# sahaRatul/sela

Hardware: AMD Instinct MI355X
Metric: Msamples/s encode+decode, 16-bit stereo 44.1kHz, 1/2/4/8 GPU; bit-exact vs CPU (higher is better)
Workload: dtype f64+int64

## Files before the change

### sela_amd/csrc/sela_encode.hip

```cpp
#include <algorithm>
#include <atomic>
#include <random>
#include <vector>

#include "sela_device.h"

namespace sela {

constexpr int kPadC = 64;
constexpr int kHalfEntries = kBlock / 4;
constexpr int kParityLen = kPadC + kHalfEntries + 64;
constexpr int kLastT0 = (kHalfEntries + 64) / 32 - 1;
constexpr int kFirstT1 = (kHalfEntries - kPadC) / 32;
constexpr int kRingHalf = 64;
constexpr int kRingLen = 2 * kRingHalf + 64;
constexpr int kRingsPerXcd = 512;
constexpr int kXcds = 8;
constexpr int kPadS = 128;
constexpr int kSBufWords = (kPadS + kBlock) / 32 * 33;
constexpr int kSmallBase = 8992;
constexpr int kBigBytes = kSmallBase + 3008;
static_assert(kResWordsCap * 4 <= kSmallBase, "packed residue words must fit the dead sample buffer");
static_assert(kSBufWords * 4 <= kSmallBase && kSmallBase % 16 == 0, "sample buffer must end below the analysis arrays");
static_assert(kBigBytes >= 2 * kParityLen * 8, "the FP64 parity arrays must fit");
// ... 877 lines not shown
    const int lane = threadIdx.x;

    const uint32_t e = blockIdx.x - n_workers;
    uint32_t frame, sig;
    block_of(e, n_sig, frame, sig);
    if (frame >= n_frames)
        return;
    const uint32_t block_id = frame * n_sig + sig;
    uint32_t flags = 0;
    if (kFused && fa.pcm_ready && !await_frame(fa.pcm_ready, pcm, frame, ticket, fa.nap_limit))
        flags |= SELA_HIP_FLAG_INTERNAL;

    double* const E = reinterpret_cast<double*>(big) + kPadC;
    double* const O = reinterpret_cast<double*>(big) + kParityLen + kPadC;
    double* const E1 = E - kHalfEntries;
    double* const O1 = O - kHalfEntries;
    SmallArrays* const sm = reinterpret_cast<SmallArrays*>(big + kSmallBase);

    int32_t s[kPerLane];
    {
        const int16_t* fp = pcm_after_wait(pcm) + (size_t)frame * kBlock * channels;
        if (channels == 2) {
            const uint32_t* fp2 = reinterpret_cast<const uint32_t*>(fp);
            uint32_t w[kPerLane];
#pragma unroll
            for (int t = 0; t < kPerLane; t++) {
                w[t] = (kFused && fa.pcm_ready) ? load_through(fp2 + lane + 64 * t) : fp2[lane + 64 * t];
            }
            unpack_stereo<kPerLane>(sig, w, s);
        } else {
            const int16_t* const ps = fp + (size_t)lane * channels + sig;
#pragma unroll
            for (int t = 0; t < kPerLane; t++)
                s[t] = ps[(uint32_t)(64 * t) * channels];
        }
    }

    double* const mine = (lane & 1) ? O : E;
    double* const mine1 = (lane & 1) ? O1 : E1;
    const int half = lane >> 1;
    double mean = 0.0;
    bool have_mean = false;
    if (e >= self_blocks) {
        for (uint32_t spin = 0; spin < kMeanWaitSpins; spin++) {
            if (__hip_atomic_load(mean_ready + e, __ATOMIC_RELAXED, __HIP_MEMORY_SCOPE_AGENT) == fa.tag) {
                __builtin_amdgcn_fence(__ATOMIC_ACQUIRE, "workgroup");
                have_mean = true;
                break;
            }
            __builtin_amdgcn_s_sleep(16);
        }
        if (have_mean)
            mean = __builtin_bit_cast(double, __hip_atomic_load(reinterpret_cast<uint64_t*>(mean_out) + e, __ATOMIC_RELAXED, __HIP_MEMORY_SCOPE_AGENT));
        have_mean = __builtin_amdgcn_readfirstlane((int)have_mean) != 0;
        mean = read_first_lane(mean);
    }
    SELA_STAMP(1);
    if (!have_mean) {
    for (int m = lane; m < kPadC; m += 64) {
        E[m - kPadC] = 0.0;
        O[m - kPadC] = 0.0;
    }
#pragma unroll
    for (int t = 0; t <= kLastT0; t++)
        mine[half + 32 * t] = scale_sample(s[t]);
    wave_sync();

    __builtin_amdgcn_s_setprio(3);
    double sum = 0.0;
#pragma unroll 1
    for (int h = 0; h < 2; h++) {
        if (h == 1) {
            wave_sync();
#pragma unroll
            for (int t = kFirstT1; t < kPerLane; t++)
                mine1[half + 32 * t] = scale_sample(s[t]);
            wave_sync();
        }
        uint32_t addr = (uint32_t)(uintptr_t)(__attribute__((address_space(3))) double*)E;
        MeanFetch f0, f1;
        SELA_MEAN_ISSUE(f0, addr, 0, sum);
#pragma unroll 1
        for (int m0 = 0; m0 < kHalfEntries; m0 += 16) {
            mean_wait(f0, sum);
            SELA_MEAN_ISSUE(f1, addr, 64, sum);
            mean_steps(f0, sum);
            mean_wait(f1, sum);
            SELA_MEAN_ISSUE(f0, addr, 128, sum);
            mean_steps(f1, sum);
            addr += 128;
        }
        mean_wait(f0, sum);
    }
    mean = sum / (double)kBlock;
    __builtin_amdgcn_s_setprio(0);
    }

    SELA_STAMP(2);
    wave_sync();
    for (int m = lane; m < kPadC; m += 64) {
        E[m - kPadC] = 0.0;
        O[m - kPadC] = 0.0;
    }
#pragma unroll
    for (int t = 0; t <= kLastT0; t++)
        mine[half + 32 * t] = scale_sample(s[t]) - mean;
    wave_sync();

    SELA_STAMP(3);
    double acc_e = 0.0, acc_o = 0.0;
    {
        uint32_t xcc;
        asm volatile("s_getreg_b32 %0, hwreg(HW_REG_XCC_ID)" : "=s"(xcc));
        xcc &= kXcds - 1;
        uint32_t* const pool = ring_owner + xcc * kRingsPerXcd;
        uint32_t slot = 0;
        if (lane == 0) {
            slot = (e >> 3) & (kRingsPerXcd - 1);
            while (atomicExch(pool + slot, ticket) == ticket)
                slot = (slot + 1) & (kRingsPerXcd - 1);
        }
        slot = (uint32_t)__builtin_amdgcn_readfirstlane((int)slot);
        double* const ring = reinterpret_cast<double*>(
            read_first_lane((uint64_t)(rings + ((size_t)xcc * kRingsPerXcd + slot) * kRingLen)));
        __attribute__((address_space(1))) double* const ring_g = (__attribute__((address_space(1))) double*)ring;
        auto store_chunk = [&](int k, const double* resident) {
#pragma unroll
            for (int t = 0; t < kRingHalf / 64; t++) {
                const double c = resident[half + 32 * (t + (kRingHalf / 64) * k)];
                ring_g[(k & 1) * kRingHalf + lane + 64 * t] = c;
                if (t == 0 && !(k & 1) && lane < 16)
                    ring_g[2 * kRingHalf + lane] = c;
            }
        };
        store_chunk(0, mine);
        store_chunk(1, mine);
        asm volatile("s_waitcnt vmcnt(0)\n\ts_dcache_inv" ::: "memory");

        double A = E[-lane];
        double B = 0.0;
        uint32_t addr_e = (uint32_t)(uintptr_t)(__attribute__((address_space(3))) double*)(E - lane);
        uint32_t addr_o = (uint32_t)(uintptr_t)(__attribute__((address_space(3))) double*)(O - lane);
        const double* c_ptr = ring;
        AcFetch f0, f1;
        asm volatile("" : "+v"(A));
        SELA_AC_ISSUE_S(f0, c_ptr, 0, 64, acc_e, acc_o);
        SELA_AC_ISSUE_V(f0, addr_e, addr_o, 0, 1, 2, 3, 4, 5, 6, 7, 8, acc_e, acc_o);
        constexpr int kSwitch = kBlock / 2 / kRingHalf;
        const bool falling = !kFused && n_workers == 0 && fa.priorities != 0;
#pragma unroll 1
        for (int k = 0; k < kBlock / kRingHalf; k++) {
            if (falling && k == 0)
                __builtin_amdgcn_s_setprio(2);
            if (falling && k == kSwitch)
                __builtin_amdgcn_s_setprio(1);
            if (k == kSwitch) {
                wave_sync();
#pragma unroll
                for (int t = kFirstT1; t < kPerLane; t++)
                    mine1[half + 32 * t] = scale_sample(s[t]) - mean;
                wave_sync();
                addr_e -= kHalfEntries * 8;
                addr_o -= kHalfEntries * 8;
            }
            if (k >= 1 && k + 1 < kBlock / kRingHalf)
                store_chunk(k + 1, k >= kSwitch ? mine1 : mine);
#pragma unroll 1
            for (int it = 0; it < kRingHalf / 32; it++) {
                if (it == kRingHalf / 32 - 1)
                    asm volatile("s_waitcnt vmcnt(0)\n\ts_dcache_inv" ::: "memory");
                ac_wait(f0, acc_e, acc_o);
                SELA_AC_ISSUE_S(f1, c_ptr, 128, 192, acc_e, acc_o);
                ac_steps_head(f0, A, B, acc_e, acc_o);
                SELA_AC_ISSUE_V(f1, addr_e, addr_o, 8, 9, 10, 11, 12, 13, 14, 15, 16, acc_e, acc_o);
                ac_steps_tail(f0, A, B, acc_e, acc_o);
                ac_wait(f1, acc_e, acc_o);
                SELA_AC_ISSUE_S(f0, c_ptr, 256, 320, acc_e, acc_o);
                ac_steps_head(f1, A, B, acc_e, acc_o);
                SELA_AC_ISSUE_V(f0, addr_e, addr_o, 16, 17, 18, 19, 20, 21, 22, 23, 24, acc_e, acc_o);
                ac_steps_tail(f1, A, B, acc_e, acc_o);
                c_ptr += 32;
                addr_e += 128;
                addr_o += 128;
            }
            if (k & 1)
                c_ptr = ring;
        }
        ac_wait(f0, acc_e, acc_o);
        if (lane == 0)
            atomicExch(pool + slot, 0u);
    }
    wave_sync();

    SELA_STAMP(4);
    {
        const double ac0 = read_first_lane(acc_e);
        if (lane <= 50) {
            sm->ac[2 * lane] = lane == 0 ? 1.0 : acc_e / ac0;
            sm->ac[2 * lane + 1] = acc_o / ac0;
        }
    }
    wave_sync();

    double k_lo = 0.0, k_hi = 0.0;
    if (!kFused && n_workers == 0 && fa.priorities != 0)
        __builtin_amdgcn_s_setprio(1);
    else
        __builtin_amdgcn_s_setprio(2);
    {
        double g0a = sm->ac[lane + 1], g1a = g0a;
        double g0b = lane < 36 ? sm->ac[lane + 65] : 0.0, g1b = g0b;
        double err = 1.0;
        double g = read_first_lane(g1a);
        double ki = -g / err;
        err += g * ki;
        sm->k[0] = ki;
        constexpr int kTwoRegs = kMaxOrder - 64 + 1;
#pragma unroll 1
        for (int i = 1; i < kTwoRegs; i++) {
            const double sa = wave_shl1(read_first_lane(g1b), g1a);
            const double sb = wave_shl1_zero(g1b);
            g1a = sa + ki * g0a;
            g0a = sa * ki + g0a;
            g1b = sb + ki * g0b;
            g0b = sb * ki + g0b;
            g = read_first_lane(g1a);
            ki = -g / err;
            err += g * ki;
            sm->k[i] = ki;
        }
#pragma unroll 1
        for (int i = kTwoRegs; i < kMaxOrder; i++) {
            const double sa = wave_shl1_zero(g1a);
            g1a = sa + ki * g0a;
            g0a = sa * ki + g0a;
            g = read_first_lane(g1a);
            ki = -g / err;
            err += g * ki;
            sm->k[i] = ki;
        }
        wave_sync();
        k_lo = sm->k[lane];
        k_hi = lane < kMaxOrder - 64 ? sm->k[lane + 64] : 0.0;
        wave_sync();
    }
    if (kMode == 3) {
        uint64_t h_ac = hash_term(sm->ac[lane], lane) ^ (lane + 64 <= kMaxOrder ? hash_term(sm->ac[lane + 64], lane + 64) : 0ull);
        uint64_t h_k = hash_term(k_lo, lane) ^ (lane < kMaxOrder - 64 ? hash_term(k_hi, lane + 64) : 0ull);
        h_ac = lanes_xor<64>(h_ac);
        h_k = lanes_xor<64>(h_k);
        if (lane == 0) {
            uint64_t* const hp = reinterpret_cast<uint64_t*>(trace) + 2 * (size_t)block_id;
            hp[0] = h_ac;
            hp[1] = h_k;
        }
    }

    {
        constexpr bool kAcInLds = true;
        uint64_t* const sizes_pub = fa.sizes_pub;
        const uint64_t sizes_tag = fa.sizes_tag;
#define SELA_TAIL_TRACE_RESIDUES fa.trace_residues
#include "sela_encode_tail.inc"
#undef SELA_TAIL_TRACE_RESIDUES
    }
    SELA_STAMP(12);
    if (kFused) {
        const uint32_t g = frame / kGroupFrames;
        const uint32_t blocks_in_group = min((uint32_t)kGroupFrames, n_frames - g * kGroupFrames) * n_sig;
        stores_done();
        uint32_t last = 0;
        if (lane == 0)
            last = group_arrive(fa.group_count + (size_t)g * kGroupCountStride, fa.tag, blocks_in_group) ? 1u : 0u;
        if (__builtin_amdgcn_readfirstlane((int)last)) {
            drop_stale_lines();
            finish_group(fa, g, lane);
        }
    }
    SELA_STAMP(13);
    if (kMode == 2 && lane == 0)
        for (int i = 0; i < 13; i++)
            phase_cycles[(size_t)block_id * 16 + i] = (uint64_t)(stamp[i + 1] - stamp[i]);
}

constexpr int kTeamMirror = 24;
constexpr int kTeamWin = 16;
constexpr int kTeamAhead = 3;
constexpr int kTeamMeanChunk = 64;

template <int P>
struct TeamPlan {
    static constexpr int B = kWave / P;
    static constexpr int G = (kMaxOrder + 1 + P - 1) / P;
    static constexpr int kChunk = P == 8 ? 16 : 64;
    static constexpr int kRing = P == 8 ? 160 : 256;
    static constexpr int kStride = P == 8 ? kRing + kTeamMirror : kRing + 48;
    static constexpr int kPer = kChunk / P;
    static constexpr int kMeanPer = kTeamMeanChunk / P;
    static constexpr int kRingBytes = B * kStride * 8;
    static constexpr int kCwBase = kBigBytes;
    static constexpr int kKStride = 104;
    static constexpr int kQBase = kSmallBase;
    static constexpr int kQStride = 104;
    static constexpr int kLdsBytes = kRingBytes > kCwBase + kCoefWordsCap * 4 ? kRingBytes : kCwBase + kCoefWordsCap * 4;
    static_assert(G + kTeamAhead <= kTeamWin && kChunk % kTeamWin == 0 && kRing % kChunk == 0 && kStride % 32 == (P == 8 ? 24 : 16) && kStride >= kRing + kTeamMirror, "team plan");
    static_assert((G * P - 1) + kChunk + kChunk <= kRing && 2 * kTeamMeanChunk <= kRing, "the ring must hold the lags' reach, the chunk in use and the chunk being written");
    static_assert(kLdsBytes * 12 <= 160 * 1024, "twelve waves per CU");
    static_assert(B * kKStride * 8 <= kQBase && B * kKStride * 8 <= kRingBytes && B * kQStride <= 104 * 8, "k[] in the dead rings below the q store; the q store inside SmallArrays::ac");
};

template <int P>
__device__ __forceinline__ uint32_t team_first(uint32_t v)
{
    if constexpr (P == 16) {
        return (uint32_t)__builtin_amdgcn_mov_dpp((int)v, 0x150 , 0xf, 0xf, true);
    } else {
        static_assert(P == 8, "teams of 8 or 16 lanes");
        const int q = __builtin_amdgcn_mov_dpp((int)v, 0x00 , 0xf, 0xf, true);
        return (uint32_t)__builtin_amdgcn_update_dpp(q, q, 0x114 , 0xf, 0xa , false);
    }
}
template <int P>
__device__ __forceinline__ double team_first(double v)
{
    const uint64_t x = __builtin_bit_cast(uint64_t, v);
    return __builtin_bit_cast(double, ((uint64_t)team_first<P>((uint32_t)(x >> 32)) << 32) | team_first<P>((uint32_t)x));
}

template <int kPer, int kStep>
__device__ __forceinline__ void team_load_raw(const int16_t* __restrict__ fp, uint32_t channels, uint32_t sig, int first, int32_t (&raw)[kPer])
{
    if (channels == 2) {
        const uint32_t* pw = reinterpret_cast<const uint32_t*>(fp) + first;
        uint32_t w[kPer];
        if constexpr (kStep == 1 && kPer % 4 == 0) {
#pragma unroll
            for (int u = 0; u < kPer / 4; u++) {
                const uint4 v = reinterpret_cast<const uint4*>(pw)[u];
                w[4 * u] = v.x, w[4 * u + 1] = v.y, w[4 * u + 2] = v.z, w[4 * u + 3] = v.w;
            }
        } else if constexpr (kStep == 1 && kPer % 2 == 0) {
#pragma unroll
            for (int u = 0; u < kPer / 2; u++) {
                const uint2 v = reinterpret_cast<const uint2*>(pw)[u];
                w[2 * u] = v.x, w[2 * u + 1] = v.y;
            }
        } else {
#pragma unroll
            for (int u = 0; u < kPer; u++)
                w[u] = pw[u * kStep];
        }
        if constexpr (kStep == 1) {
            const uint32_t first_shift = sig == 1 ? 16u : 0u;
            const uint32_t second_mask = sig == 2 ? 0xFFFFFFFFu : 0u;
#pragma unroll
            for (int i = 0; i < kPer; i++) {
                const int32_t a = (int32_t)(w[i] << (16 - first_shift)) >> 16, b = ((int32_t)w[i] >> 16) & (int32_t)second_mask;
                raw[i] = a - b;
            }
        } else {
            unpack_stereo<kPer>(sig, w, raw);
        }
    } else {
        const int16_t* const ps = fp + (size_t)first * channels + sig;
#pragma unroll
        for (int i = 0; i < kPer; i++)
            raw[i] = ps[(uint32_t)(i * kStep) * channels];
    }
}

template <int kPer, int kStep, bool kStereo>
__device__ __forceinline__ void team_fetch(const int16_t* __restrict__ fp, uint32_t channels, uint32_t sig, int first, uint32_t (&w)[kPer])
{
    if constexpr (kStereo) {
        const uint32_t* pw = reinterpret_cast<const uint32_t*>(fp) + first;
#pragma unroll
        for (int u = 0; u < kPer; u++)
            w[u] = pw[u * kStep];
    } else {
        const int16_t* const ps = fp + (size_t)first * channels + sig;
#pragma unroll
        for (int i = 0; i < kPer; i++)
            w[i] = (uint32_t)(int32_t)ps[(uint32_t)(i * kStep) * channels];
    }
}
template <int kPer, bool kStereo>
__device__ __forceinline__ void team_unpack(uint32_t sig, const uint32_t (&w)[kPer], int32_t (&raw)[kPer])
{
    if constexpr (kStereo) {
        unpack_stereo<kPer>(sig, w, raw);
    } else {
#pragma unroll
        for (int i = 0; i < kPer; i++)
            raw[i] = (int32_t)w[i];
    }
}

template <int kPer, int kStep, bool kCentre, bool kMirror, int kRing>
__device__ __forceinline__ void team_stage(double* ring_b, int pos, const int32_t (&raw)[kPer], double mean)
{
#pragma unroll
    for (int i = 0; i < kPer; i++) {
        const double x = scale_sample(raw[i]);
        const double c = kCentre ? x - mean : x;
        ring_b[pos + i * kStep] = c;
        if (kMirror && pos + i * kStep < kTeamMirror)
            ring_b[kRing + pos + i * kStep] = c;
    }
}

template <int kN>
__device__ __forceinline__ double team_chain(const double* x, double sum)
{
    constexpr int kBatch = 8;
    static_assert(kN % (2 * kBatch) == 0, "two batches per round");
    double u[kBatch], v[kBatch];
#pragma unroll
    for (int i = 0; i < kBatch; i++)
        u[i] = x[i];
#pragma unroll
    for (int i0 = 0; i0 < kN; i0 += 2 * kBatch) {
#pragma unroll
        for (int i = 0; i < kBatch; i++)
            v[i] = x[i0 + kBatch + i];
        __builtin_amdgcn_sched_barrier(0);
#pragma unroll
        for (int i = 0; i < kBatch; i++)
            sum += u[i];
        __builtin_amdgcn_sched_barrier(0);
        if (i0 + 2 * kBatch < kN) {
#pragma unroll
            for (int i = 0; i < kBatch; i++)
                u[i] = x[i0 + 2 * kBatch + i];
        }
        __builtin_amdgcn_sched_barrier(0);
#pragma unroll
        for (int i = 0; i < kBatch; i++)
            sum += v[i];
        __builtin_amdgcn_sched_barrier(0);
    }
    return sum;
}

template <int kN>
__device__ __forceinline__ double row_chain(const double (&x)[kN], double sum)
{
#define SELA_ROW_FMAC(j) "v_fmac_f64_dpp %0, %1, %2 row_newbcast:" #j "\n\t"
#pragma unroll
    for (int i = 0; i < kN; i++)
        asm("s_nop 1\n\t" SELA_ROW_FMAC(0) SELA_ROW_FMAC(1) SELA_ROW_FMAC(2) SELA_ROW_FMAC(3) SELA_ROW_FMAC(4) SELA_ROW_FMAC(5)
            SELA_ROW_FMAC(6) SELA_ROW_FMAC(7) SELA_ROW_FMAC(8) SELA_ROW_FMAC(9) SELA_ROW_FMAC(10) SELA_ROW_FMAC(11) SELA_ROW_FMAC(12)
            SELA_ROW_FMAC(13) SELA_ROW_FMAC(14) SELA_ROW_FMAC(15)
            : "+v"(sum) : "v"(x[i]), "v"(1.0));
#undef SELA_ROW_FMAC
    return sum;
}

template <int kPer, bool kStereo>
__device__ __forceinline__ double team_row_mean_sum(const int16_t* __restrict__ fp, uint32_t channels, uint32_t sig, int p)
{
    constexpr int kStep = 16, kChunks = kBlock / kTeamMeanChunk;
    static_assert(kPer * kStep == kTeamMeanChunk && kChunks % 2 == 0, "lane p holds samples p, p + 16, .. of a chunk; two chunks per trip");
    uint32_t w_a[kPer], w_b[kPer];
    double x[kPer];
    int32_t raw[kPer];
    team_fetch<kPer, kStep, kStereo>(fp, channels, sig, p, w_a);
    team_unpack<kPer, kStereo>(sig, w_a, raw);
#pragma unroll
    for (int i = 0; i < kPer; i++)
        x[i] = scale_sample(raw[i]);
    team_fetch<kPer, kStep, kStereo>(fp, channels, sig, kTeamMeanChunk + p, w_a);
    team_fetch<kPer, kStep, kStereo>(fp, channels, sig, 2 * kTeamMeanChunk + p, w_b);
    double sum = 0.0;
#pragma unroll 1
    for (int c = 0; c < kChunks; c += 2) {
        sum = row_chain<kPer>(x, sum);
        __builtin_amdgcn_sched_barrier(0);
        team_unpack<kPer, kStereo>(sig, w_a, raw);
#pragma unroll
        for (int i = 0; i < kPer; i++)
            x[i] = scale_sample(raw[i]);
        team_fetch<kPer, kStep, kStereo>(fp, channels, sig, min(c + 3, kChunks - 1) * kTeamMeanChunk + p, w_a);
        __builtin_amdgcn_sched_barrier(0);
        sum = row_chain<kPer>(x, sum);
        __builtin_amdgcn_sched_barrier(0);
        team_unpack<kPer, kStereo>(sig, w_b, raw);
#pragma unroll
        for (int i = 0; i < kPer; i++)
            x[i] = scale_sample(raw[i]);
        team_fetch<kPer, kStep, kStereo>(fp, channels, sig, min(c + 4, kChunks - 1) * kTeamMeanChunk + p, w_b);
        __builtin_amdgcn_sched_barrier(0);
    }
    return sum;
}

template <int G, int R0>
__device__ __forceinline__ void team_ac_steps(double (&W)[kTeamWin], double (&M)[4], double (&acc)[G], uint32_t addr_w, uint32_t addr_m)
{
    asm volatile("ds_read_b64 %0, %2 offset:%4\n\tds_read_b64 %1, %3 offset:%4"
                 : "=&v"(W[(R0 + kTeamAhead) & (kTeamWin - 1)]), "=&v"(M[(R0 + kTeamAhead) & 3])
                 : "v"(addr_w), "v"(addr_m), "n"(8 * (R0 + kTeamAhead)), "v"(acc[0]), "v"(acc[G - 1])
                 : "memory");
    asm volatile("s_waitcnt lgkmcnt(6)" : "+v"(W[R0 & (kTeamWin - 1)]), "+v"(M[R0 & 3]));
    const double m = M[R0 & 3];
    constexpr int kAheadOps = 5;
#pragma unroll
    for (int g0 = 0; g0 < G; g0 += kAheadOps) {
        double t[kAheadOps];
#pragma unroll
        for (int u = 0; u < kAheadOps; u++)
            if (g0 + u < G)
                t[u] = m * W[(R0 - g0 - u) & (kTeamWin - 1)];
#pragma unroll
        for (int u = 0; u < kAheadOps; u++)
            if (g0 + u < G)
                acc[g0 + u] += t[u];
    }
    __builtin_amdgcn_sched_barrier(0);
    if constexpr (R0 < kTeamWin - 1)
        team_ac_steps<G, R0 + 1>(W, M, acc, addr_w, addr_m);
}

template <int kMode, int P>
__global__ __launch_bounds__(64) __attribute__((amdgpu_waves_per_eu(3, 3))) void k_encode_teams(
    const int16_t* __restrict__ pcm, uint32_t n_frames, uint32_t channels, uint32_t n_sig, BlockMeta* __restrict__ meta,
    uint32_t* __restrict__ slots, sela_hip_trace* __restrict__ trace, int force_plain_fir, uint64_t* __restrict__ phase_cycles,
    uint64_t* __restrict__ sizes_pub, uint64_t sizes_tag, uint32_t team_priorities)
{
    using Plan = TeamPlan<P>;
    constexpr int B = Plan::B, G = Plan::G, kPer = Plan::kPer, kMeanPer = Plan::kMeanPer, kChunk = Plan::kChunk, kRing = Plan::kRing;
    constexpr bool kTrace = kMode == 1;
    constexpr bool kFused = false;
    constexpr int kStep = P == 16 ? P : 1;
    __shared__ __attribute__((aligned(32))) unsigned char lds[Plan::kLdsBytes];
    unsigned char* const big = lds;
    uint32_t* const cw_buf = reinterpret_cast<uint32_t*>(lds + Plan::kCwBase);

    const int lane0 = threadIdx.x;
    const int b = lane0 / P, p = lane0 % P;
    const uint32_t wq = blockIdx.x % 8, wv = blockIdx.x / 8;
    const uint32_t sig = wv % n_sig;
    const uint32_t frame0 = ((wv / n_sig) * 8 + wq) * B;
    constexpr uint32_t frame_stride = 1;
    if (frame0 >= n_frames)
        return;
    const bool team_live = frame0 + (uint32_t)b * frame_stride < n_frames;
    const uint32_t my_frame = team_live ? frame0 + (uint32_t)b * frame_stride : frame0;
    const int16_t* const fp = pcm + (size_t)my_frame * kBlock * channels;
    double* const ring_b = reinterpret_cast<double*>(lds) + b * Plan::kStride;
    double* const k_b = reinterpret_cast<double*>(lds) + b * Plan::kKStride;
    long long wave_stamp[5];
    if (kMode == 2)
        wave_stamp[0] = clock64();

    double mean;
    if constexpr (P == 16) {
        static_assert(kStep == P, "lane p holds samples p, p + 16, .. of a chunk");
        set_wave_priority((int)(team_priorities & 0xFF));
        const double sum = channels == 2 ? team_row_mean_sum<kMeanPer, true>(fp, channels, sig, p) : team_row_mean_sum<kMeanPer, false>(fp, channels, sig, p);
        mean = sum / (double)kBlock;
    } else {
        constexpr int kChunks = kBlock / kTeamMeanChunk;
        const int mine = kStep == 1 ? p * kMeanPer : p;
        int32_t raw_a[kMeanPer], raw_b[kMeanPer];
        team_load_raw<kMeanPer, kStep>(fp, channels, sig, mine, raw_a);
        team_stage<kMeanPer, kStep, false, false, kRing>(ring_b, mine, raw_a, 0.0);
        team_load_raw<kMeanPer, kStep>(fp, channels, sig, kTeamMeanChunk + mine, raw_a);
        team_load_raw<kMeanPer, kStep>(fp, channels, sig, 2 * kTeamMeanChunk + mine, raw_b);
        double sum = 0.0;
        const uint32_t quarter_priorities = team_priorities;
        set_wave_priority((int)(quarter_priorities & 0xFF));
#pragma unroll 1
        for (int c = 0; c < kChunks; c++) {
            const int here = (c & 1) * kTeamMeanChunk, there = kTeamMeanChunk - here;
            if (c + 1 < kChunks)
                team_stage<kMeanPer, kStep, false, false, kRing>(ring_b, there + mine, raw_a, 0.0);
#pragma unroll
            for (int i = 0; i < kMeanPer; i++)
                raw_a[i] = raw_b[i];
            if (c + 3 < kChunks)
                team_load_raw<kMeanPer, kStep>(fp, channels, sig, (c + 3) * kTeamMeanChunk + mine, raw_b);
            wave_sync();
            sum = team_chain<kTeamMeanChunk>(ring_b + here, sum);
            wave_sync();
        }
        mean = sum / (double)kBlock;
    }
    if (kMode == 2)
        wave_stamp[1] = clock64();

    double acc[G];
    {
#pragma unroll
        for (int g = 0; g < G; g++)
            acc[g] = 0.0;
        for (int i = kChunk + p; i < Plan::kStride; i += P)
            ring_b[i] = 0.0;
        const int mine = kStep == 1 ? p * kPer : p;
        int32_t raw_a[kPer], raw_b[kPer];
        team_load_raw<kPer, kStep>(fp, channels, sig, mine, raw_a);
        team_stage<kPer, kStep, true, true, kRing>(ring_b, mine, raw_a, mean);
        team_load_raw<kPer, kStep>(fp, channels, sig, kChunk + mine, raw_a);
        team_load_raw<kPer, kStep>(fp, channels, sig, 2 * kChunk + mine, raw_b);
        wave_sync();
        const uint32_t ring_addr = (uint32_t)(uintptr_t)(__attribute__((address_space(3))) double*)ring_b;
        double W[kTeamWin], M[4];
#pragma unroll
        for (int i = 0; i < kTeamWin; i++)
            W[i] = 0.0;
        uint32_t idx_w = (uint32_t)((kRing - G * p) % kRing);
        uint32_t idx_m = 0, pos_stage = kChunk;
        uint32_t addr_w = ring_addr + 8 * idx_w, addr_m = ring_addr;
        asm volatile("ds_read_b64 %0, %6\n\tds_read_b64 %3, %7\n\t"
                     "ds_read_b64 %1, %6 offset:8\n\tds_read_b64 %4, %7 offset:8\n\t"
                     "ds_read_b64 %2, %6 offset:16\n\tds_read_b64 %5, %7 offset:16"
                     : "=&v"(W[0]), "=&v"(W[1]), "=&v"(W[2]), "=&v"(M[0]), "=&v"(M[1]), "=&v"(M[2])
                     : "v"(addr_w), "v"(addr_m)
                     : "memory");
        M[3] = 0.0;
        constexpr int kChunks = kBlock / kChunk;
        auto trips = [&]() {
#pragma unroll 1
            for (int it = 0; it < kChunk / kTeamWin; it++) {
                team_ac_steps<G, 0>(W, M, acc, addr_w, addr_m);
                idx_w += kTeamWin;
                idx_w = idx_w >= (uint32_t)kRing ? idx_w - kRing : idx_w;
                idx_m += kTeamWin;
                idx_m = idx_m >= (uint32_t)kRing ? idx_m - kRing : idx_m;
                addr_w = ring_addr + 8 * idx_w;
                addr_m = ring_addr + 8 * idx_m;
            }
        };
        auto stage_next = [&](const int32_t (&raw)[kPer]) {
            team_stage<kPer, kStep, true, true, kRing>(ring_b, (int)pos_stage + mine, raw, mean);
            pos_stage += kChunk;
            pos_stage = pos_stage >= (uint32_t)kRing ? 0u : pos_stage;
        };
        constexpr int kPrio2From = (int)(0.27 * kChunks), kPrio1From = (int)(0.71 * kChunks);
#pragma unroll 1
        for (int c = 0; c < kChunks; c++) {
            if (c == kPrio2From)
                set_wave_priority((int)((team_priorities >> 8) & 0xFF));
            if (c == kPrio1From)
                set_wave_priority((int)((team_priorities >> 16) & 0xFF));
            if (c + 1 < kChunks)
                stage_next(raw_a);
#pragma unroll
            for (int i = 0; i < kPer; i++)
                raw_a[i] = raw_b[i];
            if (c + 3 < kChunks)
                team_load_raw<kPer, kStep>(fp, channels, sig, (c + 3) * kChunk + mine, raw_b);
            trips();
        }
        asm volatile("s_waitcnt lgkmcnt(0)" : "+v"(W[0]), "+v"(W[1]), "+v"(W[2]), "+v"(M[0]), "+v"(M[1]), "+v"(M[2]));
    }
    wave_sync();
    if (kMode == 2)
        wave_stamp[2] = clock64();

    {
        const double ac0 = team_first<P>(acc[0]);
#pragma unroll
        for (int g = 0; g < G; g++)
            acc[g] = (p == 0 && g == 0) ? 1.0 : acc[g] / ac0;
    }
    if (kTrace && team_live) {
        sela_hip_trace* tr = trace + (size_t)my_frame * n_sig + sig;
        if (p == 0)
            tr->mean = mean;
#pragma unroll
        for (int g = 0; g < G; g++)
            if (G * p + g <= kMaxOrder)
                tr->ac[G * p + g] = acc[g];
    }
    if (kMode == 3) {
        uint64_t h = 0;
#pragma unroll
        for (int g = 0; g < G; g++)
            h ^= G * p + g <= kMaxOrder ? hash_term(acc[g], G * p + g) : 0ull;
        h = lanes_xor<P>(h);
        if (team_live && p == 0)
            reinterpret_cast<uint64_t*>(trace)[2 * ((size_t)my_frame * n_sig + sig)] = h;
    }

    {
        double g0[G], g1[G];
        const double next_first = wave_shl1_zero(acc[0]);
#pragma unroll
        for (int r = 0; r < G; r++) {
            const double v = r + 1 < G ? acc[r + 1] : next_first;
            g0[r] = g1[r] = (G * p + r < kMaxOrder) ? v : 0.0;
        }
        double err = 1.0;
        const bool keeper = p == 0;
        double g = team_first<P>(g1[0]);
        double ki = -g / err;
        err += g * ki;
        if (keeper)
            k_b[0] = ki;
#pragma unroll 1
        for (int i = 1; i < kMaxOrder; i++) {
            const double crossing = wave_shl1_zero(g1[0]);
#pragma unroll
            for (int r = 0; r < G; r++) {
                const double sa = r + 1 < G ? g1[r + 1] : crossing;
                g1[r] = sa + ki * g0[r];
                g0[r] = sa * ki + g0[r];
            }
            g = team_first<P>(g1[0]);
            ki = -g / err;
            err += g * ki;
            if (keeper)
                k_b[i] = ki;
        }
    }
    wave_sync();
    if (kMode == 2)
        wave_stamp[3] = clock64();

    int8_t* const q_all = reinterpret_cast<int8_t*>(lds + Plan::kQBase);
#pragma unroll 1
    for (int bb = 0; bb < B; bb++) {
        const uint32_t frame = frame0 + (uint32_t)bb * frame_stride;
        if (frame >= n_frames)
            break;
        int lane_now = lane0;
        asm volatile("" : "+v"(lane_now));
        const int lane = lane_now;
        const double* const k_mine = reinterpret_cast<const double*>(lds) + bb * Plan::kKStride;
        const double k_lo = k_mine[lane];
        const double k_hi = lane < kMaxOrder - 64 ? k_mine[64 + lane] : 0.0;
        int order;
        {
            const unsigned long long b_lo = __ballot(fabs(k_lo) > SELA_ORDER_THRESHOLD);
            const unsigned long long b_hi = __ballot(lane < 36 && fabs(k_hi) > SELA_ORDER_THRESHOLD);
            order = b_hi ? 128 - __clzll(b_hi) : (b_lo ? 64 - __clzll(b_lo) : 1);
        }
        const double sqrt2 = SELA_SQRT2;
        double v_lo;
        if (lane == 0)
            v_lo = floor(64 * (-1 + (sqrt2 * sqrt(k_lo + 1))));
        else if (lane == 1)
            v_lo = floor(64 * (-1 + (sqrt2 * sqrt(-k_lo + 1))));
        else
            v_lo = floor(64 * k_lo);
        const double v_hi = floor(64 * k_hi);
        const int32_t q_lo = isnan(v_lo) ? 0 : (int32_t)v_lo;
        const int32_t q_hi = isnan(v_hi) ? 0 : (int32_t)v_hi;
        const bool wide = (lane < order && (q_lo < -128 || q_lo > 127)) || (lane + 64 < order && (q_hi < -128 || q_hi > 127));
        const bool escape = __any(wide);
        int8_t* const q_mine = q_all + bb * Plan::kQStride;
        q_mine[lane] = (int8_t)q_lo;
        if (lane < kMaxOrder - 64)
            q_mine[64 + lane] = (int8_t)q_hi;
        if (lane == 0) {
            q_mine[100] = (int8_t)order;
            q_mine[101] = escape ? 1 : 0;
        }
        if (escape) {
            int32_t* const q_wide = reinterpret_cast<int32_t*>(slots + ((size_t)frame * n_sig + sig) * kSlotWords);
            q_wide[lane] = q_lo;
            if (lane < kMaxOrder - 64)
                q_wide[64 + lane] = q_hi;
        }
        if (kTrace) {
            sela_hip_trace* tr = trace + (size_t)frame * n_sig + sig;
            tr->k[lane] = k_lo;
            if (lane < 36)
                tr->k[lane + 64] = k_hi;
        }
        if (kMode == 3) {
            uint64_t h = hash_term(k_lo, lane) ^ (lane < kMaxOrder - 64 ? hash_term(k_hi, lane + 64) : 0ull);
            h = lanes_xor<64>(h);
            if (lane == 0)
                reinterpret_cast<uint64_t*>(trace)[2 * ((size_t)frame * n_sig + sig) + 1] = h;
        }
    }
    wave_sync();

    SmallArrays* const sm = reinterpret_cast<SmallArrays*>(big + kSmallBase);
    long long stamp[14];
#pragma unroll 1
    for (int bb = 0; bb < B; bb++) {
        const uint32_t frame = frame0 + (uint32_t)bb * frame_stride;
        if (frame >= n_frames)
            break;
        int lane_now = lane0;
        asm volatile("" : "+v"(lane_now));
        const int lane = lane_now;
        const uint32_t block_id = frame * n_sig + sig;
        if (4 * (bb + 1) > B)
            set_wave_priority((int)((team_priorities >> 24) & 0xFF));
        const int8_t* const q_mine = q_all + bb * Plan::kQStride;
        const int order = (uint8_t)q_mine[100];
        int32_t q_lo = q_mine[lane], q_hi = lane < kMaxOrder - 64 ? q_mine[64 + lane] : 0;
        if (__builtin_amdgcn_readfirstlane((int)q_mine[101])) {
            const int32_t* const q_wide = reinterpret_cast<const int32_t*>(slots + (size_t)block_id * kSlotWords);
            q_lo = q_wide[lane];
            q_hi = lane < kMaxOrder - 64 ? q_wide[64 + lane] : 0;
        }
        const double mean = 0.0;
        int32_t s[kPerLane];
        {
            const int16_t* fb = pcm + (size_t)frame * kBlock * channels;
            if (channels == 2) {
                const uint32_t* fp2 = reinterpret_cast<const uint32_t*>(fb);
                uint32_t w[kPerLane];
#pragma unroll
                for (int t = 0; t < kPerLane; t++)
                    w[t] = fp2[lane + 64 * t];
                unpack_stereo<kPerLane>(sig, w, s);
            } else {
                const int16_t* const ps = fb + (size_t)lane * channels + sig;
#pragma unroll
                for (int t = 0; t < kPerLane; t++)
                    s[t] = ps[(uint32_t)(64 * t) * channels];
            }
        }
        uint32_t flags = 0;
        wave_sync();
        {
            constexpr bool kAcInLds = false;
#define SELA_TAIL_HAVE_Q
#include "sela_encode_tail.inc"
#undef SELA_TAIL_HAVE_Q
        }
        SELA_STAMP(12);
        if (kMode == 2 && lane == 0) {
            uint64_t* row = phase_cycles + (size_t)block_id * 16;
            const long long now = clock64();
            row[0] = 0;
            row[1] = (uint64_t)(wave_stamp[1] - wave_stamp[0]);
            row[2] = 0;
            row[3] = (uint64_t)(wave_stamp[2] - wave_stamp[1]);
            row[4] = (uint64_t)(wave_stamp[3] - wave_stamp[2]);
            for (int i = 5; i < 12; i++)
                row[i] = (uint64_t)(stamp[i + 1] - stamp[i]);
            row[12] = (uint64_t)(now - wave_stamp[3]);
            row[13] = (uint64_t)wave_stamp[0];
            row[14] = (uint64_t)now;
        }
    }
}

constexpr int kPlanThreadsBig = 1024, kPlanFramesBig = 12288;
constexpr int kPlanThreadsSmall = 256, kPlanFramesSmall = 4096;

template <int kPlanThreads, int kPlanLdsFrames>
__global__ __launch_bounds__(kPlanThreads) void k_plan_frames(const BlockMeta* __restrict__ meta, uint32_t n_frames,
    uint32_t channels, uint32_t n_sig, size_t frames_cap, uint64_t* frame_offsets,
    uint8_t* __restrict__ choice_out, uint32_t* __restrict__ status,
    const uint64_t* base_in ,
    uint32_t accumulate )
{
    __shared__ uint64_t part[kPlanThreads / kWave];
    __shared__ uint32_t frame_size[kPlanLdsFrames];
    __shared__ uint32_t acc[2];
    __shared__ uint64_t start;
    const uint32_t tid = threadIdx.x;
    if (tid < 2)
        acc[tid] = 0;
    if (tid == 0)
        start = base_in ? *base_in : 0;
    __syncthreads();
    uint64_t base = start;
    uint32_t flags = 0, overflow = 0;
    for (uint32_t tile0 = 0; tile0 < n_frames; tile0 += kPlanLdsFrames) {
        const uint32_t tile_n = min((uint32_t)kPlanLdsFrames, n_frames - tile0);
        __syncthreads();
#pragma unroll 8
        for (uint32_t i = tid; i < tile_n; i += kPlanThreads) {
            uint32_t choice;
            const uint32_t words = frame_words(meta + (size_t)(tile0 + i) * n_sig, channels, choice, flags);
            choice_out[tile0 + i] = (uint8_t)choice;
            frame_size[i] = (uint32_t)sela_frame_bytes(channels, words);
        }
        __syncthreads();
        const uint32_t per = (tile_n + kPlanThreads - 1) / kPlanThreads;
        const uint32_t begin = min(tid * per, tile_n), end = min(begin + per, tile_n);
        uint64_t bytes = 0;
        for (uint32_t i = begin; i < end; i++)
            bytes += frame_size[i];
        uint64_t incl = bytes;
        const int lane = (int)(tid % kWave);
#pragma unroll
        for (int d = 1; d < kWave; d <<= 1) {
            const uint32_t lo = (uint32_t)__shfl_up((int)(uint32_t)incl, d, kWave), hi = (uint32_t)__shfl_up((int)(uint32_t)(incl >> 32), d, kWave);
            if (lane >= d)
                incl += ((uint64_t)hi << 32) | lo;
        }
        if (lane == kWave - 1)
            part[tid / kWave] = incl;
        __syncthreads();
        uint64_t before = 0, tile_total = 0;
#pragma unroll
        for (int w = 0; w < kPlanThreads / kWave; w++) {
            const uint64_t t = part[w];
            before += w < (int)(tid / kWave) ? t : 0;
            tile_total += t;
        }
        __syncthreads();
        uint64_t off = base + before + incl - bytes;
        for (uint32_t i = begin; i < end; i++) {
            frame_offsets[tile0 + i] = off;
            off += frame_size[i];
            if (off > frames_cap)
                overflow++;
        }
        base += tile_total;
    }
    if (tid == 0)
        frame_offsets[n_frames] = base;
    if (flags)
        atomicOr(&acc[0], flags);
    if (overflow)
        atomicAdd(&acc[1], overflow);
    __syncthreads();
    if (tid == 0) {
        if (accumulate) {
            status[0] |= acc[0];
            status[1] += acc[1];
        } else {
            status[0] = acc[0];
            status[1] = acc[1];
            status[2] = status[3] = 0;
        }
    }
}

constexpr int kAsmThreads = 256;

__global__ __launch_bounds__(kAsmThreads) void k_assemble_frames(const BlockMeta* __restrict__ meta,
    const uint32_t* __restrict__ slots, const uint8_t* __restrict__ choice, const uint64_t* __restrict__ frame_offsets,
    uint32_t n_frames, uint32_t channels, uint32_t n_sig, size_t frames_cap, uint8_t* __restrict__ frames)
{
    const uint32_t f = blockIdx.x;
    if (f >= n_frames)
        return;
    const uint64_t begin = frame_offsets[f], end = frame_offsets[f + 1];
    if (end > frames_cap)
        return;
    uint32_t* out = reinterpret_cast<uint32_t*>(frames + begin);
    const uint32_t tid = threadIdx.x;
    if (tid == 0)
        out[0] = SELA_SYNC_WORD;
    uint32_t p = 1;
    for (uint32_t c = 0; c < channels; c++) {
        uint32_t sig = c, type = 0, parent = c;
        if (c == 1 && channels == 2 && choice[f]) {
            sig = 2;
            type = 1;
            parent = 0;
        }
        const BlockMeta b = meta[(size_t)f * n_sig + sig];
        const uint32_t* slot = slots + ((size_t)f * n_sig + sig) * kSlotWords;
        const uint32_t cw = b.coef_words, rw = b.res_words;
        if (tid == 0)
            out[p] = c | (type << 8) | (parent << 16) | ((uint32_t)b.coef_k << 24);
        for (uint32_t i = tid; i <= cw; i += kAsmThreads) {
            const uint32_t low = i == 0 ? (cw | ((uint32_t)b.order << 16)) : (slot[i - 1] >> 8);
            const uint32_t top = i < cw ? slot[i] : (uint32_t)b.res_k;
            out[p + 1 + i] = (low & 0x00FFFFFFu) | (top << 24);
        }
        if (tid == 0)
            out[p + 2 + cw] = rw | ((uint32_t)kBlock << 16);
        const uint32_t* rs = slot + kCoefWordsCap;
        uint32_t* ro = out + p + 3 + cw;
        for (uint32_t i = tid; i < rw; i += kAsmThreads)
            ro[i] = rs[i];
        p += 3 + cw + rw;
    }
}

__global__ __launch_bounds__(64) void k_stage_rice_encode(const int32_t* __restrict__ values, const uint64_t* __restrict__ value_offsets,
    uint32_t n_streams, uint32_t* __restrict__ k_out, uint32_t* __restrict__ word_counts, uint32_t* __restrict__ words_out,
    const uint64_t* __restrict__ word_offsets, uint32_t* __restrict__ status)
{
    const uint32_t s = blockIdx.x;
    if (s >= n_streams)
        return;
    const int lane = threadIdx.x;
    const int32_t* v = values + value_offsets[s];
    const uint64_t n = value_offsets[s + 1] - value_offsets[s];
    uint32_t* out = words_out + word_offsets[s];
    const uint64_t cap = word_offsets[s + 1] - word_offsets[s];
    uint64_t sum[SELA_MAX_RICE_PARAM];
#pragma unroll
    for (int k = 0; k < SELA_MAX_RICE_PARAM; k++)
        sum[k] = 0;
    bool wide = false;
    for (uint64_t i = lane; i < n; i += 64) {
        const int32_t x = v[i];
        wide |= (x >= (1 << 30)) || (x < -(1 << 30));
        const uint32_t u = zigzag32(x);
#pragma unroll
        for (int k = 0; k < SELA_MAX_RICE_PARAM; k++)
            sum[k] += u >> k;
    }
    uint32_t best_k = 0;
    uint64_t best_bits = ~0ull;
#pragma unroll
    for (int k = 0; k < SELA_MAX_RICE_PARAM; k++) {
        const uint64_t bits = wave_sum_u64(sum[k]) + n * (uint64_t)(1 + k);
        if (bits < best_bits)
            best_bits = bits, best_k = (uint32_t)k;
    }
    uint32_t flags = __any(wide) ? (uint32_t)SELA_HIP_FLAG_RICE_RANGE : 0u;
    const uint32_t words = best_bits < (1ull << 31) ? words_for_bits(best_bits) : 0xFFFFFFFFu;
    if (words > cap)
        flags |= SELA_HIP_FLAG_WORDS_CAP;
    if (lane == 0) {
        k_out[s] = best_k;
        word_counts[s] = words;
        if (flags)
            atomicOr(&status[0], flags);
    }
    if (flags)
// ... 296 lines not shown
```

Before: 17100.

## Shrink Schur recursion column count per team as columns die, repacking via LDS

The Schur (reflection coefficient) recursion in the team encoder now runs in phases for 16-lane teams: once the last column held per lane can no longer influence remaining coefficients, the g0/g1 register arrays are repacked through LDS into one fewer column per lane. Later stages then update fewer columns, which cuts the FP64 work in the serial order recursion. The cost is extra LDS stores and loads plus wave syncs at each phase boundary, along with more code from unrolling the recursive template.

```diff
diff --git a/sela_amd/csrc/sela_encode.hip b/sela_amd/csrc/sela_encode.hip
--- a/sela_amd/csrc/sela_encode.hip
+++ b/sela_amd/csrc/sela_encode.hip
@@ -1203,7 +1203,12 @@
     static constexpr int kKStride = 104;
     static constexpr int kQBase = kSmallBase;
     static constexpr int kQStride = 104;
-    static constexpr int kLdsBytes = kRingBytes > kCwBase + kCoefWordsCap * 4 ? kRingBytes : kCwBase + kCoefWordsCap * 4;
+    static constexpr int kSchurBase = B * kKStride;
+    static constexpr int kSchurStride = P == 16 ? 2 * P * G : 0;
+    static constexpr int kSchurBytes = P == 16 ? (kSchurBase + B * kSchurStride) * 8 : 0;
+    static constexpr int kTailBytes = kCwBase + kCoefWordsCap * 4;
+    static constexpr int kLdsBytes = kRingBytes > kTailBytes ? kRingBytes : kTailBytes;
+    static_assert(kSchurBytes <= kLdsBytes, "the repack areas fit the kernel's LDS");
     static_assert(G + kTeamAhead <= kTeamWin && kChunk % kTeamWin == 0 && kRing % kChunk == 0 && kStride % 32 == (P == 8 ? 24 : 16) && kStride >= kRing + kTeamMirror, "team plan");
     static_assert((G * P - 1) + kChunk + kChunk <= kRing && 2 * kTeamMeanChunk <= kRing, "the ring must hold the lags' reach, the chunk in use and the chunk being written");
     static_assert(kLdsBytes * 12 <= 160 * 1024, "twelve waves per CU");
@@ -1420,6 +1425,60 @@
     __builtin_amdgcn_sched_barrier(0);
     if constexpr (R0 < kTeamWin - 1)
         team_ac_steps<G, R0 + 1>(W, M, acc, addr_w, addr_m);
+}
+
+template <int P>
+struct TeamSchur {
+    static constexpr int G = TeamPlan<P>::G;
+    static constexpr bool kPhased = P == 16;
+    static constexpr int kFirstStage(int g) { return g >= G || !kPhased ? 1 : kMaxOrder + 1 - P * g; }
+    static constexpr int kEndStage(int g) { return g == 1 || !kPhased ? kMaxOrder : kFirstStage(g - 1); }
+};
+
+template <int P, int gFrom, int gTo>
+__device__ __forceinline__ void team_schur_repack(double (&g0)[TeamPlan<P>::G], double (&g1)[TeamPlan<P>::G], double* __restrict__ area, int p)
+{
+    double* const w = area + gFrom * p;
+    const double* const r = area + gTo * p;
+#pragma unroll
+    for (int c = 0; c < gFrom; c++) {
+        w[c] = g0[c];
+        w[P * gFrom + c] = g1[c];
+    }
+    wave_sync();
+#pragma unroll
+    for (int c = 0; c < gTo; c++) {
+        g0[c] = r[c];
+        g1[c] = r[P * gFrom + c];
+    }
+    wave_sync();
+}
+
+template <int P, int g>
+__device__ __forceinline__ void team_schur_phases(double (&g0)[TeamPlan<P>::G], double (&g1)[TeamPlan<P>::G], double& ki, double& err,
+    bool keeper, double* __restrict__ k_b, double* __restrict__ area, int p)
+{
+    using S = TeamSchur<P>;
+    static_assert(S::kFirstStage(g) >= 1 && S::kFirstStage(g) < S::kEndStage(g) && P * g - 1 >= kMaxOrder - S::kFirstStage(g), "a phase starts when its last column is dead");
+#pragma unroll 1
+    for (int i = S::kFirstStage(g); i < S::kEndStage(g); i++) {
+        const double crossing = wave_shl1_zero(g1[0]);
+#pragma unroll
+        for (int r = 0; r < g; r++) {
+            const double sa = r + 1 < g ? g1[r + 1] : crossing;
+            g1[r] = sa + ki * g0[r];
+            g0[r] = sa * ki + g0[r];
+        }
+        const double first = team_first<P>(g1[0]);
+        ki = -first / err;
+        err += first * ki;
+        if (keeper)
+            k_b[i] = ki;
+    }
+    if constexpr (S::kPhased && g > 1) {
+        team_schur_repack<P, g, g - 1>(g0, g1, area, p);
+        team_schur_phases<P, g - 1>(g0, g1, ki, err, keeper, k_b, area, p);
+    }
 }
 
 template <int kMode, int P>
@@ -1599,21 +1658,8 @@
         err += g * ki;
         if (keeper)
             k_b[0] = ki;
-#pragma unroll 1
-        for (int i = 1; i < kMaxOrder; i++) {
-            const double crossing = wave_shl1_zero(g1[0]);
-#pragma unroll
-            for (int r = 0; r < G; r++) {
-                const double sa = r + 1 < G ? g1[r + 1] : crossing;
-                g1[r] = sa + ki * g0[r];
-                g0[r] = sa * ki + g0[r];
-            }
-            g = team_first<P>(g1[0]);
-            ki = -g / err;
-            err += g * ki;
-            if (keeper)
-                k_b[i] = ki;
-        }
+        double* const area = reinterpret_cast<double*>(lds) + Plan::kSchurBase + b * Plan::kSchurStride;
+        team_schur_phases<P, G>(g0, g1, ki, err, keeper, k_b, area, p);
     }
     wave_sync();
     if (kMode == 2)
```

After: 17320, median of 6. 1.01x the previous value.
